# tobiashepp/torch-mednet

Measured on AMD Instinct MI355X. Metric: 128^3 patches/sec training, 3D U-Net 32-base-ch, higher is better.
Workload: dtype bf16; 1 GPU; ResidualUNet3D f_maps=[32, 64, 128, 256] 4-class, 128^3 patches, batch 4/GPU, fwd+DiceLoss+bwd+allreduce+Adam (BASELINE config 2); global_batch=4, parallelism=dp1, graph_replay=False, gradient_exchange=none (1 rank)

## Files before the change

include/mednet_hip.h:

```cpp
#ifndef MEDNET_HIP_H
#define MEDNET_HIP_H
#include <stddef.h>
#include <stdint.h>
#ifdef __cplusplus
extern "C" {
#endif

typedef void* mednet_stream;

enum { MEDNET_F32 = 0, MEDNET_BF16 = 1,
       MEDNET_F16 = 2,
       MEDNET_U8 = 3,
       MEDNET_I64 = 4,
       MEDNET_I16 = 5   };
enum { MEDNET_NDHWC = 0, MEDNET_NCDHW = 1 };
enum { MEDNET_ACT_NONE = 0, MEDNET_ACT_RELU = 1, MEDNET_ACT_LEAKY = 2, MEDNET_ACT_ELU = 3 };
enum { MEDNET_POOL_MAX = 0, MEDNET_POOL_AVG = 1 };
enum { MEDNET_ALGO_AUTO = 0, MEDNET_ALGO_DIRECT = 1, MEDNET_ALGO_MFMA = 2, MEDNET_ALGO_EXACT = 3,
       MEDNET_ALGO_EXACT_BIT = 4,
       MEDNET_ALGO_SPLITW_BIT = 8 };
enum { MEDNET_PACK_LOW = 0x100,
       MEDNET_PACK_HIGH_ONLY = 0x200 };
enum { MEDNET_REG_L2 = 0, MEDNET_REG_L1 = 1 };
enum { MEDNET_CLASS_DICE = 0, MEDNET_CLASS_CE = 1, MEDNET_CLASS_DICE_CE = 2 };
enum {
  MEDNET_OK = 0, MEDNET_E_SHAPE = -1, MEDNET_E_DTYPE = -2, MEDNET_E_WORKSPACE = -3, MEDNET_E_HIP = -4,
  MEDNET_E_UNSUPPORTED = -5
};
#define MEDNET_NO_IGNORE INT32_MIN

int mednet_abi_version(void);
const char* mednet_last_error(void);
int mednet_device_ok(void);
int mednet_set_option(const char* name, int value);
int mednet_get_option(const char* name, int default_value);

size_t mednet_conv3d_pack_bytes(int cin, int cout, int ksize);
int mednet_conv3d_pack_elt(const float* w, void* packed, int cin, int cout, int ksize, int transposed_src, int elt_dtype,
                           mednet_stream stream);
int mednet_conv3d_pack(const float* w, void* packed, int cin, int cout, int ksize, int transposed_src,
                       mednet_stream stream);
typedef struct mednet_pack_job {
  const float* w;
  void* packed;
  int cin, cout, ksize, transposed_src;
} mednet_pack_job;
size_t mednet_conv3d_pack_table_bytes(int njobs);
int mednet_conv3d_pack_table(const mednet_pack_job* jobs, int njobs, void* table_host, unsigned* blocks);
int mednet_conv3d_pack_many(const void* table_device, int njobs, unsigned blocks, int elt_dtype, mednet_stream stream);
int mednet_conv3d_stats_plan(int n, int d, int h, int w, int cin, int cout, int dtype, int gnb, int stride, int* out13);
int mednet_conv3d_fused_stats_chunks(int n, int d, int h, int w, int cin, int cout, int ksize, int x_dtype,
                                     int y_dtype, int algo);
int mednet_conv3d_fwd(const void* x, const void* packed, const float* bias, void* y, int n, int d, int h, int w,
                      int cin, int cout, int ksize, int x_dtype, int x_layout, int y_dtype, int y_layout,
                      int dgrad, int algo, float* gn_partial, mednet_stream stream);
int mednet_conv3d_cm_supported(int cin, int cout, int ksize, int x_dtype, int y_dtype, int algo);
int mednet_conv3d_act_supported(int n, int d, int h, int w, int cin, int cout, int algo);
int mednet_conv3d_act_fwd(const void* x, const void* packed, void* y, int n, int d, int h, int w, int cin, int cout,
                          int act, int algo, float* gn_partial, int dtype, mednet_stream stream);
int mednet_conv3d_dgrad_add(const void* dy, const void* packed, const void* add, void* dx, int n, int d, int h, int w,
                            int cin, int cout, int algo, int dtype, mednet_stream stream);
int mednet_conv3d_dgrad_gn_rows(int n, int d, int h, int w, int cin, int cout, int algo);
int mednet_conv3d_dgrad_gn_rows_dt(int n, int d, int h, int w, int cin, int cout, int algo, int dtype);
int mednet_conv3d_dgrad_add_supported(int n, int d, int h, int w, int cin, int cout, int algo, int dtype);
int mednet_conv3d_dgrad_gn(const void* dy, const void* packed, const void* add, void* dx, const void* gn_y,
                           const float* gn_coef, int gn_act, float* gn_partial, int n, int d, int h, int w, int cin,
                           int cout, int algo, int dtype, mednet_stream stream);
int mednet_head_dgrad_gn_rows(int n, int d, int h, int w, int cin, int dtype);
int mednet_head_dgrad_gn(const void* dy, const void* packed, void* dx, const void* gn_y, const void* gn_z, int gn_act,
                         float* gn_partial, int n, int d, int h, int w, int cin, int cout, int dtype, mednet_stream stream);
int mednet_convt3d_dgrad_gn_rows(int n, int d, int h, int w, int cin, int cout, int dtype, int algo);
int mednet_convt3d_dgrad_gn(const void* dy, const void* packed, void* dx, const void* gn_y, const void* gn_z, int gn_act,
                            float* gn_partial, int n, int d, int h, int w, int cin, int cout, int dtype, int algo,
                            mednet_stream stream);
int mednet_pool2_bwd_gn_rows(int n, int d, int h, int w, int c, int dtype);
int mednet_pool2_bwd_gn(const void* dy, const void* x, const void* add, void* dx, const void* gn_y, int gn_act,
                        float* gn_partial, int n, int d, int h, int w, int c, int mode, int dtype, mednet_stream stream);
size_t mednet_conv3d_wgrad_ws_bytes(int n, int d, int h, int w, int cin, int cout, int ksize, int workgroups);
int mednet_conv3d_wgrad_coresident(int n, int d, int h, int w, int cin, int cout, int ksize, int x_dtype, int dy_dtype, int algo);
int mednet_conv3d_wgrad_plan(int n, int d, int h, int w, int cin, int cout, int dtype, int workgroups, int* out10);
int mednet_conv3d_wgrad_c1_gn_supported(int cout, int x_dtype, int dtype);
int mednet_conv3d_wgrad_c1_gn(const void* x, const void* dz, const void* y, const float* coef, const float* bcoef, float* dw,
                              int n, int d, int h, int w, int cout, int act, int x_dtype, int dtype, void* ws, size_t ws_bytes,
// ... 329 lines not shown
```

torch-mednet_amd/csrc/api.hip:

```cpp
#include <stdarg.h>
#include <string.h>
#include "common.h"
#include "conv.h"

static thread_local char g_err[512] = "";

int mednet_internal_fail(int code, const char* fmt, ...) {
  va_list ap;
  va_start(ap, fmt);
  vsnprintf(g_err, sizeof(g_err), fmt, ap);
  va_end(ap);
  return code;
}
int mednet_internal_check_launch(const char* what) {
  const hipError_t e = hipGetLastError();
  if (e != hipSuccess) return mednet_internal_fail(MEDNET_E_HIP, "%s: %s", what, hipGetErrorString(e));
  return MEDNET_OK;
}

struct Option {
  char name[32];
  int value;
};
static Option g_options[48];
// ... 139 lines not shown
static int conv_common_checks(const char* who, int n, int d, int h, int w, int cin, int cout, int ksize, int dt1, int dt2) {
  MEDNET_REQUIRE(dtype_ok(dt1) && dtype_ok(dt2), MEDNET_E_DTYPE, "%s: bad dtype", who);
  MEDNET_REQUIRE(ksize == 3 || ksize == 1, MEDNET_E_UNSUPPORTED, "%s: kernel size %d (supported: 1, 3)", who, ksize);
  MEDNET_REQUIRE(n > 0 && d > 0 && h > 0 && w > 0 && cin > 0 && cout > 0, MEDNET_E_SHAPE,
                 "%s: bad shape n=%d d=%d h=%d w=%d cin=%d cout=%d", who, n, d, h, w, cin, cout);
  return MEDNET_OK;
}

extern "C" int mednet_conv3d_cm_supported(int cin, int cout, int ksize, int x_dtype, int y_dtype, int algo) {
  if (algo_base(algo) == MEDNET_ALGO_DIRECT || !is16(y_dtype) || !tuning_option("conv_cm", 1)) return 0;
  return cin >= 2 && ELT_CALL(y_dtype, conv_first_mfma_supported, cin, cout, ksize, x_dtype, y_dtype, MEDNET_NDHWC, false) ? 1 : 0;
}

extern "C" int mednet_conv3d_fused_stats_chunks(int n, int d, int h, int w, int cin, int cout, int ksize, int x_dtype,
                                                int y_dtype, int algo) {
  if (algo_base(algo) == MEDNET_ALGO_DIRECT || !tuning_option("conv_fuse_stats", 1)) return 0;
  if (x_dtype == MEDNET_F32 && y_dtype == MEDNET_F32) {
    if (!(algo_f32_mode(algo, x_dtype, y_dtype) && algo_x3(algo))) return 0;
    if (conv_c1_x3_supported(cin, cout, ksize)) return tuning_option("x3_stats", 1) ? conv_c1_x3_stats_rows(d, h, w) : 0;
    return conv_x3_supported(cin, cout, ksize) && conv_x3_fits(d, h, w, cin) ? conv_x3_stats_rows(n, d, h, w, cout) : 0;
  }
  if (cin == 1 ? ELT_CALL(y_dtype, conv_first_mfma_supported, cin, cout, ksize, x_dtype, y_dtype, MEDNET_NDHWC, false)
               : mednet_conv3d_cm_supported(cin, cout, ksize, x_dtype, y_dtype, algo))
    return ELT_CALL(y_dtype, conv_first_stats_chunks, n, d, h, w, cout);
  if (!ELT_CALL(y_dtype, conv_mfma_supported, cin, cout, ksize, x_dtype, y_dtype, MEDNET_NDHWC, MEDNET_NDHWC, false)) return 0;
  return conv_mfma_stats_chunks(n, d, h, w, cin, cout, false, algo_split(algo, y_dtype));
}

extern "C" int mednet_conv3d_stats_plan(int n, int d, int h, int w, int cin, int cout, int dtype, int gnb, int stride, int* out13) {
  MEDNET_REQUIRE(out13 && n > 0 && d > 0 && h > 0 && w > 0 && (stride == 1 || stride == 2), MEDNET_E_SHAPE, "conv3d_stats_plan: bad arguments");
  MEDNET_REQUIRE(is16(dtype) && cin % 16 == 0 && cout % 16 == 0, MEDNET_E_UNSUPPORTED,
                 "conv3d_stats_plan: the 16-bit matrix-core kernels only (dtype %d, %d -> %d)", dtype, cin, cout);
  return ELT_CALL(dtype, conv_mfma_plan, n, d, h, w, cin, cout, (gnb & 1) != 0, stride, out13, (gnb & 2) != 0);
}

extern "C" int mednet_conv3d_fwd(const void* x, const void* packed, const float* bias, void* y, int n, int d, int h,
                                 int w, int cin, int cout, int ksize, int x_dtype, int x_layout, int y_dtype,
                                 int y_layout, int dgrad, int algo, float* gn_partial, mednet_stream stream) {
  int rc = conv_common_checks("conv3d_fwd", n, d, h, w, cin, cout, ksize, x_dtype, y_dtype);
  if (rc) return rc;
  const PackLayout L = dgrad ? pack_layout(cout, cin, ksize) : pack_layout(cin, cout, ksize);
  hipStream_t s = (hipStream_t)stream;
  const bool mfma_ok = ELT_CALL(y_dtype, conv_mfma_supported, cin, cout, ksize, x_dtype, y_dtype, x_layout, y_layout, bias != nullptr) &&
                       conv_mfma_fits(n, d, h, w, cin);
  const bool f32_mode = algo_f32_mode(algo, x_dtype, y_dtype) && ksize == 3 && (x_layout == MEDNET_NDHWC || cin == 1) && y_layout == MEDNET_NDHWC;
  if (!dgrad && !bias && y_layout == MEDNET_NDHWC && (x_layout == MEDNET_NDHWC || x_layout == MEDNET_NCDHW) &&
      mednet_conv3d_cm_supported(cin, cout, ksize, x_dtype, y_dtype, algo))
    return ELT_CALL(y_dtype, launch_conv_first_mfma, x, x_layout, x_dtype, pack_f32(packed, L, 0), y, n, d, h, w, cin, cout,
                    gn_partial, s, algo_split(algo, y_dtype) ? 1 : 0);
  if (algo_base(algo) == MEDNET_ALGO_MFMA && !mfma_ok && !f32_mode)
    return fail(MEDNET_E_UNSUPPORTED, "conv3d_fwd: MFMA path does not take cin=%d cout=%d k=%d dtypes %d->%d", cin, cout,
                ksize, x_dtype, y_dtype);
  if (mfma_ok && algo_base(algo) != MEDNET_ALGO_DIRECT)
    return ELT_CALL(y_dtype, launch_conv_mfma, x, pack_mfma(packed, L, dgrad), y, n, d, h, w, cin, cout, x_dtype,
                    y_dtype, gn_partial, s, MEDNET_ACT_NONE, nullptr, algo_lo_delta(algo, y_dtype, L));
  if (!dgrad && algo_base(algo) != MEDNET_ALGO_DIRECT && x_layout == MEDNET_NDHWC && cin == 1 &&
      ELT_CALL(y_dtype, conv_first_mfma_supported, cin, cout, ksize, x_dtype, y_dtype, y_layout, bias != nullptr))
    return ELT_CALL(y_dtype, launch_conv_first_mfma, x, x_layout, x_dtype, pack_f32(packed, L, 0), y, n, d, h, w, cin, cout,
                    gn_partial, s, algo_split(algo, y_dtype) ? 1 : 0);
  if (f32_mode && algo_x3(algo) && L.mfma_bytes && conv_x3_supported(cin, cout, ksize) && conv_x3_fits(d, h, w, cin))
    return launch_conv_x3(x, pack_mfma(packed, L, dgrad), L.lo_delta, bias, y, n, d, h, w, cin, cout, gn_partial, s);
  if (f32_mode && !dgrad && algo_x3(algo) && conv_c1_x3_supported(cin, cout, ksize))
    return launch_conv_c1_x3(x, pack_f32(packed, L, 0), bias, y, n, d, h, w, cout, gn_partial, s);
  MEDNET_REQUIRE(gn_partial == nullptr, MEDNET_E_UNSUPPORTED,
                 "conv3d_fwd: fused GroupNorm partials are only produced by the MFMA paths (ask mednet_conv3d_fused_stats_chunks)");
  if (f32_mode)
// ... 527 lines not shown
```

torch-mednet_amd/csrc/conv_mfma.hip:

```cpp
#include <type_traits>
#include "conv.h"

#include "elt16.inc"

namespace mednet {

template <int KIND>
struct FwdTile;
template <>
struct FwdTile<1> {
  static constexpr int TZ = 4, TY = 8, TX = 16, STRIDE = 1;
};
template <>
struct FwdTile<2> {
  static constexpr int TZ = 2, TY = 4, TX = 16, STRIDE = 2;
};
template <>
struct FwdTile<3> {
  static constexpr int TZ = 4, TY = 8, TX = 8, STRIDE = 1;
};
static bool narrow_bricks(int w) {
  const int mode = tuning_option("conv_narrow", 1);
  return mode != 0 && (w <= 8 || (mode == 2 && (w + 7) / 8 < 2 * ((w + 15) / 16)));
}
// ... 444 lines not shown
      for (int k = 0; k < 8; ++k) {
        park[k * 256] = ebs[k];
        park[(8 + k) * 256] = ebq[k];
      }
    }
    if (a.gn_partial && !a.stats_accum) flush_any(n, tis * 4 + e_wv, cb);
    if (!has_next) {
      if (a.gn_partial && a.stats_accum) {
        while (acc_n < a.n) {
          flush_any(acc_n, acc_row, cb);
          ++acc_n;
        }
      }
      break;
    }
    cur_bid = nbid;
    ctile = ntile;
    ccb = ncb2;
  }
}

enum : int { C32_GNB = 1, C32_ADD = 2, C32_STATS = 4, C32_ACT = 8, C32_SPLIT = 16  };
#ifdef MEDNET_ELT_F16
#define MEDNET_MFMA_ASM_OP "v_mfma_f32_32x32x16_f16"
#else
#define MEDNET_MFMA_ASM_OP "v_mfma_f32_32x32x16_bf16"
#endif
__device__ __forceinline__ void mfma_a_acc(f32x16& acc, const eltx8& w_in_agpr, const eltx8& b) {
  asm volatile(MEDNET_MFMA_ASM_OP " %0, %1, %2, %0" : "+v"(acc) : "a"(w_in_agpr), "v"(b));
}
__device__ __forceinline__ void mfma_a_zero(f32x16& acc, const eltx8& w_in_agpr, const eltx8& b) {
  asm volatile(MEDNET_MFMA_ASM_OP " %0, %1, %2, 0" : "=v"(acc) : "a"(w_in_agpr), "v"(b));
}
template <int V>
__global__ __launch_bounds__(256, 1) void conv32_mfma_kernel(FwdArgs a) {
  constexpr bool GNB = (V & C32_GNB) != 0, ADD = (V & C32_ADD) != 0, STATS = (V & C32_STATS) != 0, ACT = (V & C32_ACT) != 0;
  static_assert(!(GNB && (STATS || ACT)), "the data-gradient variant has its own sums and no activation");
  constexpr int TZ = 4, TY = 8, TX = 16, HZ = 6, HY = 10, HX = 18, NV = HZ * HY * HX, NTW = 4;
  constexpr int PIECES = 4 * NV, IN_ROUNDS = (PIECES + 255) / 256;
  constexpr int NVP = NV + 4, BUF_PIECES = 4 * NVP;
  typedef __attribute__((ext_vector_type(4))) unsigned u32x4;
  typedef __attribute__((ext_vector_type(2))) elt eltx2;
  extern __shared__ __attribute__((aligned(16))) char smem[];
  u32x4* in_lds = reinterpret_cast<u32x4*>(smem);
  elt* wlds = reinterpret_cast<elt*>(smem + (size_t)2 * BUF_PIECES * 16) + (threadIdx.x >> 6) * 2048;
  const int tid = threadIdx.x, lane = tid & 63, wv = tid >> 6;
  const int r = lane & 31, h = lane >> 5;
  const int wv_s = __builtin_amdgcn_readfirstlane(wv);
  const int xcd = (int)(blockIdx.x & 7);
  auto origin = [&](int q, int& n, int& tz0, int& ty0, int& tx0) {
    if (a.zslab) {
      int qd = fastdiv(q, a.tiles_x, a.rcp_tiles_x);
      tx0 = (q - qd * a.tiles_x) * TX;
      const int yy = fastdiv(qd, a.zslab, a.rcp_zslab);
      const int zz = xcd * a.zslab + (qd - yy * a.zslab);
      ty0 = yy * TY;
      n = fastdiv(zz, a.tiles_z, a.rcp_tiles_z);
      tz0 = (zz - n * a.tiles_z) * TZ;
    } else {
      int tt = a.xcd_chunk ? xcd * a.xcd_chunk + q : q;
      int qd = fastdiv(tt, a.tiles_x, a.rcp_tiles_x);
      tx0 = (tt - qd * a.tiles_x) * TX;
      tt = qd;
      qd = fastdiv(tt, a.tiles_y, a.rcp_tiles_y);
      ty0 = (tt - qd * a.tiles_y) * TY;
      tt = qd;
      qd = fastdiv(tt, a.tiles_z, a.rcp_tiles_z);
// ... 45 lines not shown
  };
  const int seq_step = a.xcd_chunk ? (int)(gridDim.x >> 3) : (int)gridDim.x;
  const int seq_end = a.xcd_chunk ? a.xcd_chunk : a.ntiles;
  int seq = a.xcd_chunk ? (int)(blockIdx.x >> 3) : (int)blockIdx.x;
  if (seq >= seq_end) {
    if constexpr (GNB || STATS)
      for (int nn = 0; nn < a.n; ++nn) flush(nn);
    return;
  }

#ifndef MEDNET_C32_GNB_LDS
#define MEDNET_C32_GNB_LDS 1
#endif
  constexpr bool GNB_LDS = GNB && MEDNET_C32_GNB_LDS;
  constexpr int NSEC = (ADD ? 8 : 0) + (GNB && !GNB_LDS ? 8 : 0);
  constexpr int SEC0 = 54 - 8, WT = NSEC, TW1 = SEC0, TW0 = TW1 - WT;
  eltx8 wreg[54];
  const u32x4* wp = reinterpret_cast<const u32x4*>(a.wpk) + h * 32 + r;
#pragma unroll
  for (int i = 0; i < 54; ++i)
    if (i < TW0 || i >= TW1) wreg[i] = __builtin_bit_cast(eltx8, wp[((i / 27) * 27 + tap_at(i % 27)) * 64]);

  constexpr unsigned OOB = 0xFFFFFF00u;
  constexpr int MAIN_ROUNDS = HZ * HY / 4, TAIL_ROUNDS = 2;
  static_assert(MAIN_ROUNDS * 4 == HZ * HY && MAIN_ROUNDS + TAIL_ROUNDS == IN_ROUNDS && TAIL_ROUNDS * 32 >= HZ * HY, "round layout");
  const int q4 = lane & 3, hx_main = lane >> 2;
  int tail_pos[TAIL_ROUNDS];
#pragma unroll
  for (int k = 0; k < TAIL_ROUNDS; ++k) {
    const int row = 32 * k + (tid >> 3);
    tail_pos[k] = row < HZ * HY ? ((row / HY) << 8) | (row % HY) : 0x7F00;
  }
  const int tail_hx = 16 + ((tid >> 2) & 1);
  u32x4 in_reg[IN_ROUNDS];
  auto rsrc_of = [&](int n, bool ok) {
    return __builtin_amdgcn_make_buffer_rsrc((void*)(a.x + (size_t)n * a.id * a.ih * a.iw * 32), 0, a.bytes_x & (0u - (unsigned)ok), 0x00020000);
  };
  unsigned voff_main = 0;
  auto plan_main = [&](int tx0) {
    const int gx = tx0 - 1 + hx_main;
    voff_main = (unsigned)gx < (unsigned)a.iw ? (unsigned)gx * 64u + (unsigned)q4 * 16u : OOB;
  };
  auto tail_voff = [&](int k, int tz0, int ty0, int tx0) {
    const int gz = tz0 - 1 + (tail_pos[k] >> 8), gy = ty0 - 1 + (tail_pos[k] & 255), gxt = tx0 - 1 + tail_hx;
    const bool ok = ((unsigned)gz < (unsigned)a.id) & ((unsigned)gy < (unsigned)a.ih) & ((unsigned)gxt < (unsigned)a.iw);
    return ok ? (unsigned)((gz * a.ih + gy) * a.iw + gxt) * 64u + (unsigned)q4 * 16u : OOB;
  };
  int lr_gz = 0, lr_gy = 0;
  unsigned lr_soff = 0, lr_num = 0;
  auto load_round = [&](int it, int phase, int n, int tz0, int ty0, int tx0, bool valid) {
    if (it < MAIN_ROUNDS) {
      if (phase == 0 || phase < 0) {
        const int row = it * 4 + wv_s;
        const int hz = (row * 205) >> 11, hy = row - hz * HY;
        lr_gz = tz0 - 1 + hz;
        lr_gy = ty0 - 1 + hy;
      }
      if (phase == 1 || phase < 0) {
        const bool ok = valid & ((unsigned)lr_gz < (unsigned)a.id) & ((unsigned)lr_gy < (unsigned)a.ih);
        lr_num = a.bytes_x & (0u - (unsigned)ok);
      }
      if (phase == 2 || phase < 0) lr_soff = (unsigned)((lr_gz * a.ih + lr_gy) * a.iw) * 64u;
      if (phase == 3 || phase < 0)
        in_reg[it] = __builtin_amdgcn_raw_buffer_load_b128(
            __builtin_amdgcn_make_buffer_rsrc((void*)(a.x + (size_t)n * a.id * a.ih * a.iw * 32), 0, lr_num, 0x00020000), voff_main, lr_soff, 0);
    } else if (phase == 3 || phase < 0) {
      in_reg[it] = __builtin_amdgcn_raw_buffer_load_b128(rsrc_of(n, valid), tail_voff(it - MAIN_ROUNDS, tz0, ty0, tx0), 0, 0);
    }
  };
  const int slot_main = q4 * NVP + hx_main;
  int slot_tail[TAIL_ROUNDS];
#pragma unroll
  for (int k = 0; k < TAIL_ROUNDS; ++k) {
    const int row = 32 * k + (tid >> 3);
    slot_tail[k] = row < HZ * HY ? q4 * NVP + row * HX + tail_hx : -1;
  }
  const int spare_slot = (2 * BUF_PIECES * 16 + 4 * 4096) / 16 + tid;
  auto commit_one = [&](int b, int it) {
    if (it < MAIN_ROUNDS) {
      in_lds[b * BUF_PIECES + (it * 4 + wv_s) * HX + slot_main] = in_reg[it];
    } else {
      const int sl = slot_tail[it - MAIN_ROUNDS];
      in_lds[sl >= 0 ? b * BUF_PIECES + sl : spare_slot] = in_reg[it];
    }
  };
  const int lx6 = ((r & 15) + 8 * (r >> 4)) & 15;
  const int lbase6 = (wv * HY + 4 * (r >> 4)) * HX + lx6;
  [[maybe_unused]] const eltx2 ones = {(elt)1.0f, (elt)1.0f};
  const size_t ovol = (size_t)a.od * a.oh * a.ow;

  {
    int n0, tz0, ty0, tx0;
    origin(seq, n0, tz0, ty0, tx0);
    plan_main(tx0);
#pragma unroll
    for (int it = 0; it < IN_ROUNDS; ++it) load_round(it, -1, n0, tz0, ty0, tx0, true);
#pragma unroll
    for (int it = 0; it < IN_ROUNDS; ++it) commit_one(0, it);
    const bool valid1 = seq + seq_step < seq_end;
    origin(valid1 ? seq + seq_step : 0, n0, tz0, ty0, tx0);
    plan_main(tx0);
#pragma unroll
    for (int it = 0; it < IN_ROUNDS; ++it) load_round(it, -1, n0, tz0, ty0, tx0, valid1);
  }
  int buf = 0;
  [[maybe_unused]] int coef_n = -1;
  [[maybe_unused]] char* cf_lds = smem + (size_t)2 * BUF_PIECES * 16 + 4 * 4096 + wv_s * 256;
  static_assert(4 * 256 <= 224 * 16, "the coefficient copies stay clear of the spare slots in use");
  while (true) {
    int n, tz0, ty0, tx0;
    origin(seq, n, tz0, ty0, tx0);
    const bool has_next = seq + seq_step < seq_end;
    const bool has_next2 = seq + 2 * seq_step < seq_end;
    if constexpr (GNB || STATS) {
      while (acc_n < n) {
        flush(acc_n);
        ++acc_n;
      }
    }
    if constexpr (GNB) {
      if (n != coef_n) {
        coef_n = n;
        const auto rsrc_cf = __builtin_amdgcn_make_buffer_rsrc((void*)(a.gnb_coef + (size_t)n * 64), 0, 256u, 0x00020000);
        const u32x4 c4 = __builtin_amdgcn_raw_buffer_load_b128(rsrc_cf, (unsigned)(lane * 16), 0, 0);
        wave_lds_fence();
        if (lane < 16) *reinterpret_cast<u32x4*>(cf_lds + lane * 16) = c4;
        wave_lds_fence();
      }
    }
    int n2, tz2, ty2, tx2;
    origin(has_next2 ? seq + 2 * seq_step : 0, n2, tz2, ty2, tx2);
    __syncthreads();

    const int pj = lane & 3, ev = lane >> 2;
    const bool plane_ok = tz0 + wv_s < a.od;
    const bool lane_ok = tx0 + ev < a.ow;
    const unsigned vb = lane_ok ? (unsigned)(ev * 32 + pj * 8) * 2u : OOB;
    unsigned row_num[8], row_off[8];
    auto plan_row = [&](int j) {
      const bool ok = plane_ok & (ty0 + j < a.oh);
      row_num[j] = a.bytes_y & (0u - (unsigned)ok);
      row_off[j] = (unsigned)((((tz0 + wv_s) * a.oh + ty0 + j) * a.ow + tx0) * 32) * 2u;
      asm volatile("" : "+s"(row_num[j]), "+s"(row_off[j]));
    };
    auto row_rsrc = [&](const elt* base, int j) {
      return __builtin_amdgcn_make_buffer_rsrc((void*)(base + (size_t)n * ovol * 32), 0, row_num[j], 0x00020000);
    };
    auto row_soff = [&](int j) { return row_off[j]; };
    [[maybe_unused]] eltx8 adr[ADD ? 8 : 1], yrw[GNB ? 8 : 1];
    [[maybe_unused]] char* ydst = reinterpret_cast<char*>(in_lds + (size_t)buf * BUF_PIECES) + wv_s * 8192;
    static_assert(!GNB_LDS || 4 * 8192 <= 2 * NVP * 16, "the four waves' rows fit the two dead planes");

    f32x16 acc[NTW];
    const u32x4* img = in_lds + (size_t)buf * BUF_PIECES;
    auto b_fragment = [&](int gq, int a6) {
      const int kc1 = gq / 9, kz1 = (gq / 3) % 3, kx1 = gq % 3;
      return __builtin_bit_cast(eltx8, img[(2 * kc1 + h) * NVP + lbase6 + (kz1 * HY + a6) * HX + kx1]);
    };
    eltx8 xf[2][6];
#pragma unroll
    for (int a6 = 0; a6 < 6; ++a6) xf[0][a6] = b_fragment(0, a6);
#pragma unroll
    for (int s54 = 0; s54 < 54; ++s54) {
      const int gq = s54 / 3, ky = s54 % 3, cur = gq & 1;
      const int round = s54 / 3;
      const bool staging = s54 % 3 == 0 && round < IN_ROUNDS;
#pragma unroll
      for (int t = 0; t < NTW; ++t) {
        __builtin_amdgcn_sched_barrier(0);
        if (s54 == 0) mfma_a_zero(acc[t], wreg[0], xf[cur][t]);
        else mfma_a_acc(acc[t], wreg[s54], xf[cur][t + ky]);
        __builtin_amdgcn_sched_barrier(0);
        if (gq + 1 < 18 && (t & 1) == 0) xf[cur ^ 1][(ky * 4 + t) >> 1] = b_fragment(gq + 1, (ky * 4 + t) >> 1);
        if (s54 == 0 && t == 1) plan_main(tx2);
        if (t == 3 && s54 >= 24 && s54 < 32) plan_row(s54 - 24);
        if (t == 2 && s54 < WT)
          wreg[TW0 + s54] = __builtin_bit_cast(eltx8, __builtin_nontemporal_load(wp + (((TW0 + s54) / 27) * 27 + tap_at((TW0 + s54) % 27)) * 64));
        if (t == 2 && s54 >= SEC0) {
          const int j = s54 - SEC0;
          if constexpr (ADD) adr[j] = __builtin_bit_cast(eltx8, __builtin_amdgcn_raw_buffer_load_b128(row_rsrc(a.add, j), vb, row_soff(j), 0));
          if constexpr (GNB && !GNB_LDS) yrw[j] = __builtin_bit_cast(eltx8, __builtin_amdgcn_raw_buffer_load_b128(row_rsrc(a.gnb_y, j), vb, row_soff(j), 0));
        }
        if constexpr (GNB_LDS) {
          if (t == 2 && s54 == 27) __builtin_amdgcn_s_barrier();
          if (t == 2 && s54 >= 27 && s54 < 35) {
            const int j = s54 - 27;
            const __amdgpu_buffer_rsrc_t yr = __builtin_amdgcn_make_buffer_rsrc((void*)(a.gnb_y + (size_t)n * ovol * 32), 0, row_num[j], 0x00020000);
            __builtin_amdgcn_raw_ptr_buffer_load_lds(yr, (__attribute__((address_space(3))) void*)(ydst + j * 1024), 16, vb, row_off[j], 0, 0);
          }
        }
        if (staging) {
          if (t == 0) commit_one(buf ^ 1, round);
          load_round(round, t, n2, tz2, ty2, tx2, has_next2);
        }
      }
    }
    __builtin_amdgcn_sched_barrier(0);

    if constexpr (ACT) {
#pragma unroll
      for (int t = 0; t < NTW; ++t) act_apply_v16(acc[t], a.act);
    }
    const int e_lx = lx6;
    const int e_sw = (e_lx >> 1) & 7;
    eltx8 rows[8];
#pragma unroll
    for (int half = 0; half < 2; ++half) {
      wave_lds_fence();
      if ((r >> 4) == half) {
#pragma unroll
        for (int t = 0; t < NTW; ++t) {
          const int vl = t * 16 + e_lx;
#pragma unroll
          for (int q = 0; q < 4; ++q) {
            eltx4 o;
#pragma unroll
            for (int j = 0; j < 4; ++j) o[j] = (elt)acc[t][q * 4 + j];
            *reinterpret_cast<eltx4*>(wlds + vl * 32 + ((2 * q + h) ^ e_sw) * 4) = o;
          }
        }
      }
      wave_lds_fence();
#pragma unroll
      for (int j = 0; j < 4; ++j) {
        const int vox = j * 16 + ev, swl = (vox >> 1) & 7;
        rows[4 * half + j] = *reinterpret_cast<const eltx8*>(wlds + vox * 32 + (pj ^ (swl >> 1)) * 8);
// ... 395 lines not shown
  const size_t fwd_bytes = mfma ? align_up((size_t)27 * ((cout + 31) / 32 * 32) * cin * sizeof(elt), 256) : 0;
  const size_t bwd_bytes = mfma ? align_up((size_t)27 * ((cin + 31) / 32 * 32) * cout * sizeof(elt), 256) : 0;
  L.mfma_bytes = fwd_bytes > bwd_bytes ? fwd_bytes : bwd_bytes;
  L.mfma_fwd = 2 * f32;
  L.mfma_bwd = 2 * f32 + fwd_bytes;
  L.lo_delta = fwd_bytes + bwd_bytes;
  L.total = 2 * f32 + 2 * (fwd_bytes + bwd_bytes) + 256;
  return L;
}

unsigned pack_mfma_blocks(int cin, int cout) { return 2 * pack_img_tiles(cin, cout); }
int launch_pack_mfma(const float* w, void* sec_fwd, void* sec_bwd, float* Pf, float* Pb, int cin, int cout, int T,
                     int transposed_src, hipStream_t s, size_t lo_delta) {
  if (T != 27) return MEDNET_OK;
  hipLaunchKernelGGL(pack_mfma_kernel, dim3(pack_mfma_blocks(cin, cout)), dim3(256), 0, s, w, (elt*)sec_fwd, (elt*)sec_bwd, cout, cin,
                     transposed_src ? 2 : 0, transposed_src ? 3 : 1, Pf, Pb, transposed_src, lo_delta);
  return check_launch("pack_mfma");
}
int launch_pack_mfma_many(const void* table_device, int njobs, unsigned max_blocks, hipStream_t s, int with_low) {
  hipLaunchKernelGGL(pack_mfma_many_kernel, dim3(max_blocks), dim3(256), 0, s, (const PackJobDev*)table_device, njobs, with_low);
  return check_launch("pack_mfma_many");
}

bool conv_mfma_fits(int n, int d, int h, int w, int c) {
  (void)n;
  return (double)d * h * w * c * 2.0 < 4294960000.0;
}
bool conv_mfma_supported(int cin, int cout, int ksize, int x_dtype, int y_dtype, int x_layout, int y_layout, bool bias) {
  return ksize == 3 && cin % 16 == 0 && cout % 16 == 0 && x_dtype == ELT_DTYPE && y_dtype == ELT_DTYPE &&
         x_layout == MEDNET_NDHWC && y_layout == MEDNET_NDHWC && !bias;
}

static bool conv32_applies(int ntiles, int cin, int cout) {
  return cin == 32 && cout == 32 && ntiles >= 512 && ::mednet_internal_cu_count() == 256 && tuning_option("conv32", 1);
}
static bool conv32_takes(int ntiles, int cin, int cout, bool gnb, bool split = false) {
  return !split && conv32_applies(ntiles, cin, cout) && (!gnb || tuning_option("conv32_gnb", 1));
}
static bool conv2b_takes(int ntiles, int cin, int cout, bool split = false) {
  if (split) return cout % 32 == 0 && cin % 16 == 0 && ::mednet_internal_cu_count() == 256 && tuning_option("conv2b_split", 1);
  if (!(cout % 64 == 0 && cin % 16 == 0 && cin >= tuning_option("conv2b_min_cin", 64) && ::mednet_internal_cu_count() == 256 &&
        tuning_option("conv2b", 1)))
    return false;
  const int nitems = ((ntiles + 7) / 8) * 8 * (cout / 64);
  const int rounds = (nitems + 255) / 256;
  return nitems >= 256 && nitems * 100 >= tuning_option("conv2b_min_fill", 80) * rounds * 256;
}
static int conv_fwd_kind(int n, int d, int h, int w, int cin, int cout, bool gnb, bool split = false) {
  return narrow_bricks(w) && !conv32_takes(bricks<FwdTile<1>>(n, d, h, w), cin, cout, gnb, split) ? 3 : 1;
}
static int conv2b_grid(int nitems) { return nitems < 256 ? nitems : 256; }
static bool convt_dgrad32_takes(int ntiles, int k_dy, int m_dx, bool split) {
  return k_dy == 32 && m_dx == 64 && !split && ntiles >= 256 && ::mednet_internal_cu_count() == 256 && tuning_option("convt_dgrad32", 1);
}
static void conv_stats_plan(int n, int d, int h, int w, int cin, int cout, int& rows, int& accum, bool gnb = false, bool split = false) {
  const int tx = conv_fwd_kind(n, d, h, w, cin, cout, gnb, split) == 3 ? FwdTile<3>::TX : FwdTile<1>::TX;
  using G = FwdTile<1>;
  const int tps = bricks<G>(1, d, h, w, tx);
  const int ncb = (cout + 31) / 32, ntiles = n * tps;
  if (tx == G::TX && conv32_takes(ntiles, cin, cout, gnb, split)) {
    accum = 1;
    rows = 256 * 4;
    return;
  }
  if (tx == G::TX && conv2b_takes(ntiles, cin, cout, split)) {
    const int ncbp = split ? cout / 32 : cout / 64;
    const int grid = conv2b_grid(((ntiles + 7) / 8) * 8 * ncbp);
    accum = tuning_option("conv_stats_accum", 1) && ntiles % 8 == 0 && (grid / 8) % ncbp == 0;
// ... 92 lines not shown
  a.rcp_zslab = 0;
  if constexpr (KIND == 2) {
    if (convt_dgrad32_takes(a.ntiles, cin, cout, split) && !add && act == MEDNET_ACT_NONE) {
      Ct32Args c;
      c.dy = a.x; c.wpk = a.wpk; c.dx = a.y;
      c.gn_y = a.gnb_y; c.gn_z = a.gnb_z; c.gn_partial = a.gn_partial; c.gn_act = a.gnb_act;
      c.n = n; c.d = od; c.h = oh; c.w = ow;
      c.tiles_z = a.tiles_z; c.tiles_y = a.tiles_y; c.tiles_x = a.tiles_x; c.ntiles = a.ntiles;
      c.rcp_tiles_x = a.rcp_tiles_x; c.rcp_tiles_y = a.rcp_tiles_y; c.rcp_tiles_z = a.rcp_tiles_z;
      c.bytes_dy = a.bytes_x; c.bytes_dx = a.bytes_y;
      const int rows32 = 2 * 256;
      if (probe) {
        a.stats_accum = 1;
        a.stats_rows = rows32;
        a.xcd_chunk = a.ntiles % 8 == 0 ? a.ntiles / 8 : 0;
        return plan_answer(probe, 7, 256, a.ntiles, a);
      }
      return launch_lds("convt_dgrad32_mfma", use_gnb ? convt_dgrad32_mfma_kernel<true> : convt_dgrad32_mfma_kernel<false>, dim3(256), dim3(256),
                        CT32_LDS, s, c);
    }
  }
  if constexpr (KIND == 1) {
    const int variant = c32_variant(use_gnb, add != nullptr, gn_partial != nullptr, act != MEDNET_ACT_NONE, split);
    if (conv32_takes(a.ntiles, cin, cout, use_gnb, split)) {
      constexpr size_t lds32 = (size_t)2 * 4 * (HZ * HY * HX + 4) * 16 + 4 * 4096 + 256 * 16;
      static_assert(lds32 <= 160 * 1024, "two bricks of whole rows + the waves' epilogue areas + spare slots");
      a.xcd_chunk = a.ntiles % 8 == 0 ? a.ntiles / 8 : 0;
      if ((n * a.tiles_z) % 8 == 0 && a.tiles_z % (n * a.tiles_z / 8) == 0 && tuning_option("conv32_zslab", 1)) {
        a.zslab = n * a.tiles_z / 8;
        a.rcp_zslab = fastdiv_rcp(a.zslab);
      }
      MEDNET_REQUIRE(!use_gnb || act == MEDNET_ACT_NONE, MEDNET_E_UNSUPPORTED, "conv32_mfma: no activation in the data-gradient form");
      if (probe) return plan_answer(probe, 4, 256, a.ntiles, a);
      return c32_dispatch(variant, [&](auto v) {
        return launch_lds("conv32_mfma", conv32_mfma_kernel<decltype(v)::value>, dim3(256), dim3(256), lds32, s, a);
      });
    }
    if (conv2b_takes(a.ntiles, cin, cout, split)) {
      FwdArgs b2 = a;
      b2.ncb = split ? cout / 32 : cout / 64;
      b2.rcp_ncb = fastdiv_rcp(b2.ncb);
      b2.nitems = ((a.ntiles + 7) / 8) * 8 * b2.ncb;
      b2.nkc = a.nkc_in;
      b2.xcd_chunk = (a.ntiles % 8 == 0 && tuning_option("conv2b_xcd_walk", 1)) ? a.ntiles / 8 : 0;
      const int grid2 = conv2b_grid(b2.nitems);
      MEDNET_REQUIRE(!use_gnb || act == MEDNET_ACT_NONE, MEDNET_E_UNSUPPORTED, "conv2b_mfma: no activation in the data-gradient form");
      if (probe) return plan_answer(probe, b2.stats_accum ? 6 : 5, grid2, b2.nitems, b2);
      return c32_dispatch(variant, [&](auto v) {
        constexpr int V = decltype(v)::value;
        return launch_lds("conv2b_mfma", split ? conv2b_mfma_kernel<V | C32_SPLIT> : conv2b_mfma_kernel<V>, dim3(grid2), dim3(256), C2B_LDS, s, b2);
      });
    }
  }
  if (probe) return plan_answer(probe, a.stats_accum ? 3 : 2, (int)grid, a.nitems, a);
  if constexpr (STRIDE == 1) {
    if (use_gnb) {
      constexpr size_t lds_gnb = lds + 16 * 256 * sizeof(float);
      static_assert(lds_gnb <= 80 * 1024, "two workgroups must fit one CU");
      return launch_lds("conv_mfma(gnb)", conv_mfma_kernel<KIND, true>, dim3(grid), dim3(256), lds_gnb, s, a);
    }
  }
  if constexpr (STRIDE == 2) {
    if (use_gnb) return launch_lds("conv_mfma(gnb, stride 2)", conv_mfma_kernel<2, true>, dim3(grid), dim3(256), lds, s, a);
  }
  return launch_lds("conv_mfma", conv_mfma_kernel<KIND>, dim3(grid), dim3(256), lds, s, a);
}

static int fwd_by_kind(const void* x, const void* sec, void* y, int n, int d, int h, int w, int cin, int cout, float* gn_partial,
// ... 10 lines not shown
  return fwd_by_kind(x, packed_section, y, n, d, h, w, cin, cout, gn_partial, s, act, add, GnbSpec(), nullptr, lo_delta);
}
int launch_conv_mfma_gnb(const void* dy, const void* packed_section, void* dx, int n, int d, int h, int w, int cin, int cout,
                         const void* add, const void* gn_y, const float* gn_coef, int gn_act, float* gn_partial, hipStream_t s,
                         size_t lo_delta) {
  GnbSpec g;
  g.y = gn_y;
  g.coef = gn_coef;
  g.act = gn_act;
  return fwd_by_kind(dy, packed_section, dx, n, d, h, w, cin, cout, gn_partial, s, MEDNET_ACT_NONE, add, g, nullptr, lo_delta);
}
int conv_mfma_plan(int n, int d, int h, int w, int cin, int cout, bool gnb, int stride, int* out, bool split) {
  FwdPlanProbe p{};
  const size_t lo = split ? 256 : 0;
  float dummy_partial;
  GnbSpec g;
  int rc;
  if (stride == 2) {
    g.y = g.z = &dummy_partial;
    rc = launch_fwd<2>(nullptr, nullptr, nullptr, n, d, h, w, 2 * d, 2 * h, 2 * w, cout, cin, &dummy_partial, nullptr, MEDNET_ACT_NONE,
                       nullptr, g, &p, lo);
  } else {
    if (gnb) {
      g.y = &dummy_partial;
      g.coef = &dummy_partial;
    }
    rc = fwd_by_kind(nullptr, nullptr, nullptr, n, d, h, w, cin, cout, &dummy_partial, nullptr, MEDNET_ACT_NONE, nullptr, g, &p, lo);
  }
  if (rc) return rc;
  const int v[13] = {p.kind, p.grid, p.nitems, p.ncb, p.ntiles, p.tiles_per_sample, p.accum, p.rows, p.xcd_chunk, p.zslab,
                     p.tiles_x, p.tiles_y, p.tiles_z};
  for (int i = 0; i < 13; ++i) out[i] = v[i];
  return MEDNET_OK;
}
int conv_mfma_stats_chunks(int n, int d, int h, int w, int cin, int cout, bool gnb, bool split) {
  int rows, accum;
  conv_stats_plan(n, d, h, w, cin, cout, rows, accum, gnb, split);
  if (gnb && !tuning_option("conv_fuse_gnb_general", 1) && !conv32_takes(bricks<FwdTile<1>>(n, d, h, w), cin, cout, true, split)) return 0;
  return rows;
}

int launch_convt_dgrad_mfma(const void* dy, const void* packed_section, void* dx, int n, int d, int h, int w, int cin,
                            int cout, hipStream_t s, size_t lo_delta) {
  return launch_fwd<2>(dy, packed_section, dx, n, d, h, w, 2 * d, 2 * h, 2 * w, cout, cin, nullptr, s, MEDNET_ACT_NONE, nullptr, GnbSpec(),
                       nullptr, lo_delta);
}
int convt_dgrad_gn_rows(int n, int d, int h, int w, int cin, int cout, bool split) {
  const int tps = bricks<FwdTile<2>>(1, d, h, w);
  if (convt_dgrad32_takes(n * tps, cout, cin, split)) return 2 * 256;
  return 4 * tps;
}
int launch_convt_dgrad_gn_mfma(const void* dy, const void* packed_section, void* dx, const void* gn_y, const void* gn_z, int gn_act,
                               float* gn_partial, int n, int d, int h, int w, int cin, int cout, hipStream_t s, size_t lo_delta) {
  GnbSpec g;
  g.y = gn_y;
  g.z = gn_z;
  g.act = gn_act;
  return launch_fwd<2>(dy, packed_section, dx, n, d, h, w, 2 * d, 2 * h, 2 * w, cout, cin, gn_partial, s, MEDNET_ACT_NONE, nullptr, g,
                       nullptr, lo_delta);
}

struct Wg2Args {
  const elt* A;
  const elt* B;
  float* part;
  int n, d, h, w, ka, kb;
// ... 725 lines not shown
```

torch-mednet_amd/csrc/conv_mfma_decl.inc:

```
struct PackLayout {
  int taps;
  size_t f32_fwd, f32_bwd;
  size_t mfma_fwd, mfma_bwd;
  size_t mfma_bytes;
  size_t lo_delta;
  size_t total;
};
PackLayout pack_layout(int cin, int cout, int ksize);
struct PackJobDev {
  const float* w;
  void* sec_fwd;
  void* sec_bwd;
  float* Pf;
  float* Pb;
  int cin, cout, transposed;
  unsigned nblocks;
  int lo_delta;
  unsigned first_block;
};
bool conv_mfma_fits(int n, int d, int h, int w, int c);
bool conv_mfma_supported(int cin, int cout, int ksize, int x_dtype, int y_dtype, int x_layout, int y_layout, bool bias);
int launch_conv_mfma(const void* x, const void* packed_section, void* y, int n, int d, int h, int w, int cin, int cout,
                     int x_dtype, int y_dtype, float* gn_partial, hipStream_t s, int act = MEDNET_ACT_NONE,
                     const void* add = nullptr, size_t lo_delta = 0);
int launch_conv_mfma_gnb(const void* dy, const void* packed_section, void* dx, int n, int d, int h, int w, int cin, int cout,
                         const void* add, const void* gn_y, const float* gn_coef, int gn_act, float* gn_partial, hipStream_t s,
                         size_t lo_delta = 0);
int conv_mfma_plan(int n, int d, int h, int w, int cin, int cout, bool gnb, int stride, int* out, bool split = false);
int conv_mfma_stats_chunks(int n, int d, int h, int w, int cin, int cout, bool gnb = false, bool split = false);
int launch_pack_mfma(const float* w, void* sec_fwd, void* sec_bwd, float* Pf, float* Pb, int cin, int cout, int T,
                     int transposed_src, hipStream_t s, size_t lo_delta = 0);
unsigned pack_mfma_blocks(int cin, int cout);
int launch_pack_mfma_many(const void* table_device, int njobs, unsigned max_blocks, hipStream_t s, int with_low = 0);
bool wgrad_mfma_supported(int cin, int cout, int ksize, int x_dtype, int dy_dtype, int x_layout, int dy_layout);
bool wgrad_mfma_fits(int n, int d, int h, int w, int cmax, int scale);
bool wgrad_mfma_coresident(int d, int h, int w);
int wgrad_mfma_plan(int n, int d, int h, int w, int cin, int cout, int workgroups, int* out);
size_t wgrad_mfma_ws_bytes(int n, int d, int h, int w, int cin, int cout, int ksize, int workgroups);
int launch_wgrad_mfma(const void* x, const void* dy, float* dw, int n, int d, int h, int w, int cin, int cout, int dtype,
                      void* ws, size_t ws_bytes, hipStream_t s, int workgroups);
int launch_convt_fwd_mfma(const void* x, const void* sec, const float* bias, const void* skip, void* y, int n, int d,
                          int h, int w, int cin, int cout, hipStream_t s, size_t lo_delta = 0);
int launch_convt_dgrad_mfma(const void* dy, const void* packed_section, void* dx, int n, int d, int h, int w, int cin,
                            int cout, hipStream_t s, size_t lo_delta = 0);
int convt_dgrad_gn_rows(int n, int d, int h, int w, int cin, int cout, bool split = false);
int launch_convt_dgrad_gn_mfma(const void* dy, const void* packed_section, void* dx, const void* gn_y, const void* gn_z, int gn_act,
                               float* gn_partial, int n, int d, int h, int w, int cin, int cout, hipStream_t s, size_t lo_delta = 0);
size_t convt_wgrad_mfma_ws_bytes(int n, int d, int h, int w, int cin, int cout, int workgroups);
int launch_convt_wgrad_mfma(const void* x, const void* dy, float* dw, int n, int d, int h, int w, int cin, int cout,
                            void* ws, size_t ws_bytes, hipStream_t s, int workgroups);

bool conv_first_mfma_supported(int cin, int cout, int ksize, int x_dtype, int y_dtype, int y_layout, bool bias);
int conv_first_stats_chunks(int n, int d, int h, int w, int cout);
int launch_conv_first_mfma(const void* x, int x_layout, int x_dtype, const float* w_pf, void* y, int n, int d, int h, int w, int cin,
                           int cout, float* gn_partial, hipStream_t s, int split = 0);
bool wgrad_first_mfma_supported(int cin, int cout, int x_dtype, int dy_dtype);
void wgrad_first_mfma_plan(int n, int d, int h, int w, int cin, int cout, bool gn, int* out4);
int wgrad_first_mfma_blocks(int n, int d, int h, int w, int cin, int cout, bool gn);
int launch_wgrad_first_mfma(const void* x, int x_layout, int x_dtype, const void* dy, float* part, int n, int d, int h, int w, int cin,
                            int cout, hipStream_t s, const void* gn_y = nullptr, const float* gn_coef = nullptr,
                            const float* gn_bcoef = nullptr, int gn_act = 0);
// ... 33 lines not shown
```

torch-mednet_amd/mednet_hip/_lib.py:

```python
from __future__ import annotations

import ctypes as C
import os

import torch

_HERE = os.path.dirname(os.path.abspath(__file__))
LIB_PATH = os.environ.get("MEDNET_LIB_PATH") or os.path.join(_HERE, "libmednet_hip.so")

F32, BF16 = 0, 1
NDHWC, NCDHW = 0, 1
ACT_NONE, ACT_RELU, ACT_LEAKY, ACT_ELU = 0, 1, 2, 3
POOL_MAX, POOL_AVG = 0, 1
ALGO_AUTO, ALGO_DIRECT, ALGO_MFMA, ALGO_EXACT = 0, 1, 2, 3
ALGO_EXACT_BIT = 4
ALGO_SPLITW_BIT = 8
PACK_LOW = 0x100
PACK_HIGH_ONLY = 0x200
REG_L2, REG_L1 = 0, 1
CLASS_DICE, CLASS_CE, CLASS_DICE_CE = 0, 1, 2
PAD_CONSTANT, PAD_SYMMETRIC = 0, 1
MIP_MEAN, MIP_MAX = 0, 1
BLEND_PROBABILITIES, BLEND_LOGITS = 0, 1
INTERP_LINEAR, INTERP_NEAREST = 0, 1
BORDER_CONSTANT, BORDER_EDGE = 0, 1
F16, U8, I64 = 2, 3, 4
I16 = 5
INTENSITY_MAX_RANKS, INTENSITY_TABLE_BYTES = 8, 40
INTENSITY_ALL, INTENSITY_FIRST, INTENSITY_LAST = -1, 1, 2
INTENSITY_ZSCORE, INTENSITY_CT, INTENSITY_RESCALE, INTENSITY_PERCENTILES = 0, 1, 2, 3
NO_IGNORE = -(2 ** 31)
CC_ALL = -1

_vp, _i, _sz, _f, _i64, _dbl = C.c_void_p, C.c_int, C.c_size_t, C.c_float, C.c_int64, C.c_double

SIGNATURES = {
    "mednet_abi_version": (_i, []),
    "mednet_last_error": (C.c_char_p, []),
    "mednet_device_ok": (_i, []),
    "mednet_set_option": (_i, [C.c_char_p, _i]),
    "mednet_get_option": (_i, [C.c_char_p, _i]),
    "mednet_conv3d_pack_bytes": (_sz, [_i, _i, _i]),
    "mednet_conv3d_pack": (_i, [_vp, _vp, _i, _i, _i, _i, _vp]),
    "mednet_conv3d_pack_elt": (_i, [_vp, _vp, _i, _i, _i, _i, _i, _vp]),
    "mednet_conv3d_pack_table_bytes": (_sz, [_i]),
    "mednet_conv3d_pack_table": (_i, [_vp, _i, _vp, _vp]),
    "mednet_conv3d_pack_many": (_i, [_vp, _i, C.c_uint, _i, _vp]),
    "mednet_conv3d_stats_plan": (_i, [_i] * 9 + [_vp]),
    "mednet_conv3d_fused_stats_chunks": (_i, [_i] * 10),
    "mednet_conv3d_fwd": (_i, [_vp, _vp, _vp, _vp] + [_i] * 13 + [_vp, _vp]),
    "mednet_gn_finalize": (_i, [_vp, _i, _vp, _vp, _vp, _vp, _i, _sz, _i, _i, _f, _vp, _sz, _vp]),
    "mednet_conv3d_act_supported": (_i, [_i] * 7),
    "mednet_conv3d_act_fwd": (_i, [_vp, _vp, _vp] + [_i] * 8 + [_vp, _i, _vp]),
    "mednet_conv3d_dgrad_add": (_i, [_vp, _vp, _vp, _vp] + [_i] * 8 + [_vp]),
    "mednet_conv3d_dgrad_gn_rows": (_i, [_i] * 7),
    "mednet_conv3d_dgrad_gn_rows_dt": (_i, [_i] * 8),
    "mednet_conv3d_dgrad_add_supported": (_i, [_i] * 8),
    "mednet_conv3d_dgrad_gn": (_i, [_vp, _vp, _vp, _vp, _vp, _vp, _i, _vp] + [_i] * 8 + [_vp]),
    "mednet_gn_act_bwd_fused": (_i, [_vp] * 6 + [_i, _vp, _vp, _vp, _i, _sz, _i, _i, _i, _i, _i, _vp, _sz, _vp]),
    "mednet_gn_bwd_coefficients": (_i, [_vp, _vp, _vp, _i, _vp, _vp, _vp, _i, _sz, _i, _i, _vp, _sz, _vp]),
    "mednet_gn_act_bwd_fused_res": (_i, [_vp] * 7 + [_i, _vp, _vp, _vp, _vp, _i, _sz, _i, _i, _i, _i, _vp, _sz, _vp]),
    "mednet_gn_act_bwd_fused_res_pool": (_i, [_vp] * 7 + [_i, _vp, _vp, _vp, _vp] + [_i] * 9 + [_vp, _sz, _vp]),
    "mednet_gn_act_bwd_fused_res_head_supported": (_i, [_i] * 4),
    "mednet_gn_act_bwd_fused_res_head": (_i, [_vp, _vp, _i, _i64] + [_vp] * 4 + [_f, _i, _i, _i, _i] + [_vp] * 5 + [_i, _vp, _vp, _vp, _vp,
                                              _i, _sz, _i, _i, _i, _i, _vp, _sz, _vp]),
    "mednet_head_dgrad_gn_rows": (_i, [_i] * 6),
    "mednet_head_dgrad_gn": (_i, [_vp] * 5 + [_i, _vp] + [_i] * 7 + [_vp]),
    "mednet_pool2_bwd_gn_rows": (_i, [_i] * 6),
    "mednet_convt3d_dgrad_gn_rows": (_i, [_i] * 8),
    "mednet_convt3d_dgrad_gn": (_i, [_vp] * 5 + [_i, _vp] + [_i] * 8 + [_vp]),
    "mednet_pool2_bwd_gn": (_i, [_vp] * 5 + [_i, _vp] + [_i] * 7 + [_vp]),
    "mednet_conv3d_wgrad_ws_bytes": (_sz, [_i] * 8),
    "mednet_conv3d_wgrad_coresident": (_i, [_i] * 10),
    "mednet_conv3d_wgrad_plan": (_i, [_i] * 8 + [_vp]),
    "mednet_conv3d_wgrad_c1_gn_supported": (_i, [_i] * 3),
    "mednet_conv3d_wgrad_c1_gn": (_i, [_vp] * 6 + [_i] * 8 + [_vp, _sz, _vp]),
    "mednet_conv3d_cm_supported": (_i, [_i] * 6),
    "mednet_conv3d_wgrad_cm_gn_supported": (_i, [_i] * 4),
    "mednet_conv3d_wgrad_cm_plan": (_i, [_i] * 8 + [_vp]),
    "mednet_conv3d_wgrad_cm_gn": (_i, [_vp, _i] + [_vp] * 5 + [_i] * 9 + [_vp, _sz, _vp]),
    "mednet_conv3d_wgrad": (_i, [_vp, _vp, _vp, _vp] + [_i] * 13 + [_vp, _sz, _vp]),
# ... 190 lines not shown
```

Baseline: 212.0 patches/s.

## Stage conv32 input halo tiles via direct buffer-to-LDS loads

Adds a DMA variant of the 32->32 channel MFMA conv kernel that loads input halo bricks straight into LDS with buffer_load_lds instead of going through registers and explicit LDS stores. Halo bounds are handled by a packed-coordinate guard test that sends out-of-range lanes to an OOB offset. Prefetch depth drops from two tiles ahead to one, with a vmcnt wait before the barrier. The variant is on by default through a tuning option. The intent is to cut VGPR pressure and LDS store instructions, at the cost of less prefetch lookahead.

```diff
diff --git a/include/mednet_hip.h b/include/mednet_hip.h
--- a/include/mednet_hip.h
+++ b/include/mednet_hip.h
@@ -49,6 +49,7 @@
 int mednet_conv3d_pack_table(const mednet_pack_job* jobs, int njobs, void* table_host, unsigned* blocks);
 int mednet_conv3d_pack_many(const void* table_device, int njobs, unsigned blocks, int elt_dtype, mednet_stream stream);
 int mednet_conv3d_stats_plan(int n, int d, int h, int w, int cin, int cout, int dtype, int gnb, int stride, int* out13);
+int mednet_conv32_form(int n, int d, int h, int w, int dtype, int gnb);
 int mednet_conv3d_fused_stats_chunks(int n, int d, int h, int w, int cin, int cout, int ksize, int x_dtype,
                                      int y_dtype, int algo);
 int mednet_conv3d_fwd(const void* x, const void* packed, const float* bias, void* y, int n, int d, int h, int w,
diff --git a/torch-mednet_amd/csrc/api.hip b/torch-mednet_amd/csrc/api.hip
--- a/torch-mednet_amd/csrc/api.hip
+++ b/torch-mednet_amd/csrc/api.hip
@@ -195,6 +195,11 @@
   MEDNET_REQUIRE(is16(dtype) && cin % 16 == 0 && cout % 16 == 0, MEDNET_E_UNSUPPORTED,
                  "conv3d_stats_plan: the 16-bit matrix-core kernels only (dtype %d, %d -> %d)", dtype, cin, cout);
   return ELT_CALL(dtype, conv_mfma_plan, n, d, h, w, cin, cout, (gnb & 1) != 0, stride, out13, (gnb & 2) != 0);
+}
+
+extern "C" int mednet_conv32_form(int n, int d, int h, int w, int dtype, int gnb) {
+  MEDNET_REQUIRE(n > 0 && d > 0 && h > 0 && w > 0 && is16(dtype), MEDNET_E_SHAPE, "conv32_form: bad arguments");
+  return ELT_CALL(dtype, conv32_form, n, d, h, w, gnb != 0);
 }
 
 extern "C" int mednet_conv3d_fwd(const void* x, const void* packed, const float* bias, void* y, int n, int d, int h,
diff --git a/torch-mednet_amd/csrc/conv_mfma.hip b/torch-mednet_amd/csrc/conv_mfma.hip
--- a/torch-mednet_amd/csrc/conv_mfma.hip
+++ b/torch-mednet_amd/csrc/conv_mfma.hip
@@ -500,7 +500,7 @@
 __device__ __forceinline__ void mfma_a_zero(f32x16& acc, const eltx8& w_in_agpr, const eltx8& b) {
   asm volatile(MEDNET_MFMA_ASM_OP " %0, %1, %2, 0" : "=v"(acc) : "a"(w_in_agpr), "v"(b));
 }
-template <int V>
+template <int V, bool DMA>
 __global__ __launch_bounds__(256, 1) void conv32_mfma_kernel(FwdArgs a) {
   constexpr bool GNB = (V & C32_GNB) != 0, ADD = (V & C32_ADD) != 0, STATS = (V & C32_STATS) != 0, ACT = (V & C32_ACT) != 0;
   static_assert(!(GNB && (STATS || ACT)), "the data-gradient variant has its own sums and no activation");
@@ -612,7 +612,7 @@
     tail_pos[k] = row < HZ * HY ? ((row / HY) << 8) | (row % HY) : 0x7F00;
   }
   const int tail_hx = 16 + ((tid >> 2) & 1);
-  u32x4 in_reg[IN_ROUNDS];
+  [[maybe_unused]] u32x4 in_reg[DMA ? 1 : IN_ROUNDS];
   auto rsrc_of = [&](int n, bool ok) {
     return __builtin_amdgcn_make_buffer_rsrc((void*)(a.x + (size_t)n * a.id * a.ih * a.iw * 32), 0, a.bytes_x & (0u - (unsigned)ok), 0x00020000);
   };
@@ -642,10 +642,10 @@
       }
       if (phase == 2 || phase < 0) lr_soff = (unsigned)((lr_gz * a.ih + lr_gy) * a.iw) * 64u;
       if (phase == 3 || phase < 0)
-        in_reg[it] = __builtin_amdgcn_raw_buffer_load_b128(
+        in_reg[DMA ? 0 : it] = __builtin_amdgcn_raw_buffer_load_b128(
             __builtin_amdgcn_make_buffer_rsrc((void*)(a.x + (size_t)n * a.id * a.ih * a.iw * 32), 0, lr_num, 0x00020000), voff_main, lr_soff, 0);
     } else if (phase == 3 || phase < 0) {
-      in_reg[it] = __builtin_amdgcn_raw_buffer_load_b128(rsrc_of(n, valid), tail_voff(it - MAIN_ROUNDS, tz0, ty0, tx0), 0, 0);
+      in_reg[DMA ? 0 : it] = __builtin_amdgcn_raw_buffer_load_b128(rsrc_of(n, valid), tail_voff(it - MAIN_ROUNDS, tz0, ty0, tx0), 0, 0);
     }
   };
   const int slot_main = q4 * NVP + hx_main;
@@ -658,10 +658,42 @@
   const int spare_slot = (2 * BUF_PIECES * 16 + 4 * 4096) / 16 + tid;
   auto commit_one = [&](int b, int it) {
     if (it < MAIN_ROUNDS) {
-      in_lds[b * BUF_PIECES + (it * 4 + wv_s) * HX + slot_main] = in_reg[it];
+      in_lds[b * BUF_PIECES + (it * 4 + wv_s) * HX + slot_main] = in_reg[DMA ? 0 : it];
     } else {
       const int sl = slot_tail[it - MAIN_ROUNDS];
-      in_lds[sl >= 0 ? b * BUF_PIECES + sl : spare_slot] = in_reg[it];
+      in_lds[sl >= 0 ? b * BUF_PIECES + sl : spare_slot] = in_reg[DMA ? 0 : it];
+    }
+  };
+  constexpr unsigned DGUARD = 0x00808080u;
+  [[maybe_unused]] unsigned dpos[DMA ? IN_ROUNDS : 1], drel[DMA ? IN_ROUNDS : 1];
+  if constexpr (DMA) {
+#pragma unroll
+    for (int k = 0; k < IN_ROUNDS; ++k) {
+      const int v = (64 * k < NV - 64 ? 64 * k : NV - 64) + lane;
+      const int hz = v / (HY * HX), hy = (v / HX) % HY, hx = v % HX;
+      dpos[k] = (unsigned)((hz << 16) | (hy << 8) | hx);
+      drel[k] = (unsigned)((hz * a.ih + hy) * a.iw + hx) * 64u + (unsigned)wv * 16u;
+    }
+  }
+  [[maybe_unused]] unsigned d_lo = 0, d_hi = 0, d_off = 0, d_num = 0, d_t = 0, d_voff = 0;
+  [[maybe_unused]] int d_n = 0;
+  auto plan_dma = [&](int n, int tz0, int ty0, int tx0, bool valid) {
+    const int zlo = tz0 < 1 ? 1 - tz0 : 0, ylo = ty0 < 1 ? 1 - ty0 : 0, xlo = tx0 < 1 ? 1 - tx0 : 0;
+    const int zhi = a.id - tz0 < HZ - 1 ? a.id - tz0 : HZ - 1, yhi = a.ih - ty0 < HY - 1 ? a.ih - ty0 : HY - 1,
+              xhi = a.iw - tx0 < HX - 1 ? a.iw - tx0 : HX - 1;
+    d_lo = (unsigned)(((128 - zlo) << 16) | ((128 - ylo) << 8) | (128 - xlo));
+    d_hi = (unsigned)(((128 + zhi) << 16) | ((128 + yhi) << 8) | (128 + xhi));
+    d_off = (unsigned)(((tz0 - 1) * a.ih + (ty0 - 1)) * a.iw + (tx0 - 1)) * 64u;
+    d_num = a.bytes_x & (0u - (unsigned)valid);
+    d_n = n;
+  };
+  auto dma_round = [&](int it, int phase, int b) {
+    if (phase == 0 || phase < 0) d_t = (dpos[DMA ? it : 0] + d_lo) & (d_hi - dpos[DMA ? it : 0]) & DGUARD;
+    if (phase == 1 || phase < 0) d_voff = d_t == DGUARD ? drel[DMA ? it : 0] + d_off : OOB;
+    if (phase == 3 || phase < 0) {
+      const __amdgpu_buffer_rsrc_t xr = __builtin_amdgcn_make_buffer_rsrc((void*)(a.x + (size_t)d_n * a.id * a.ih * a.iw * 32), 0, d_num, 0x00020000);
+      char* dst = smem + (size_t)(((b * 4 + wv_s) * NVP + (64 * it < NV - 64 ? 64 * it : NV - 64)) * 16);
+      __builtin_amdgcn_raw_ptr_buffer_load_lds(xr, (__attribute__((address_space(3))) void*)dst, 16, d_voff, 0, 0, 0);
     }
   };
   const int lx6 = ((r & 15) + 8 * (r >> 4)) & 15;
@@ -669,7 +701,13 @@
   [[maybe_unused]] const eltx2 ones = {(elt)1.0f, (elt)1.0f};
   const size_t ovol = (size_t)a.od * a.oh * a.ow;
 
-  {
+  if constexpr (DMA) {
+    int n0, tz0, ty0, tx0;
+    origin(seq, n0, tz0, ty0, tx0);
+    plan_dma(n0, tz0, ty0, tx0, true);
+#pragma unroll
+    for (int it = 0; it < IN_ROUNDS; ++it) dma_round(it, -1, 0);
+  } else {
     int n0, tz0, ty0, tx0;
     origin(seq, n0, tz0, ty0, tx0);
     plan_main(tx0);
@@ -709,7 +747,13 @@
       }
     }
     int n2, tz2, ty2, tx2;
-    origin(has_next2 ? seq + 2 * seq_step : 0, n2, tz2, ty2, tx2);
+    if constexpr (DMA) {
+      origin(has_next ? seq + seq_step : 0, n2, tz2, ty2, tx2);
+      plan_dma(n2, tz2, ty2, tx2, has_next);
+      asm volatile("s_waitcnt vmcnt(0)" ::: "memory");
+    } else {
+      origin(has_next2 ? seq + 2 * seq_step : 0, n2, tz2, ty2, tx2);
+    }
     __syncthreads();
 
     const int pj = lane & 3, ev = lane >> 2;
@@ -752,7 +796,7 @@
         else mfma_a_acc(acc[t], wreg[s54], xf[cur][t + ky]);
         __builtin_amdgcn_sched_barrier(0);
         if (gq + 1 < 18 && (t & 1) == 0) xf[cur ^ 1][(ky * 4 + t) >> 1] = b_fragment(gq + 1, (ky * 4 + t) >> 1);
-        if (s54 == 0 && t == 1) plan_main(tx2);
+        if (!DMA && s54 == 0 && t == 1) plan_main(tx2);
         if (t == 3 && s54 >= 24 && s54 < 32) plan_row(s54 - 24);
         if (t == 2 && s54 < WT)
           wreg[TW0 + s54] = __builtin_bit_cast(eltx8, __builtin_nontemporal_load(wp + (((TW0 + s54) / 27) * 27 + tap_at((TW0 + s54) % 27)) * 64));
@@ -770,8 +814,12 @@
           }
         }
         if (staging) {
-          if (t == 0) commit_one(buf ^ 1, round);
-          load_round(round, t, n2, tz2, ty2, tx2, has_next2);
+          if constexpr (DMA) {
+            dma_round(round, t, buf ^ 1);
+          } else {
+            if (t == 0) commit_one(buf ^ 1, round);
+            load_round(round, t, n2, tz2, ty2, tx2, has_next2);
+          }
         }
       }
     }
@@ -1233,8 +1281,10 @@
 }
 
 static bool conv32_applies(int ntiles, int cin, int cout) {
-  return cin == 32 && cout == 32 && ntiles >= 512 && ::mednet_internal_cu_count() == 256 && tuning_option("conv32", 1);
-}
+  return cin == 32 && cout == 32 && ntiles >= tuning_option("conv32_min_bricks", 512) && ::mednet_internal_cu_count() == 256 &&
+         tuning_option("conv32", 1);
+}
+static bool conv32_dma() { return tuning_option("conv32_dma", 1) != 0; }
 static bool conv32_takes(int ntiles, int cin, int cout, bool gnb, bool split = false) {
   return !split && conv32_applies(ntiles, cin, cout) && (!gnb || tuning_option("conv32_gnb", 1));
 }
@@ -1393,8 +1443,10 @@
       }
       MEDNET_REQUIRE(!use_gnb || act == MEDNET_ACT_NONE, MEDNET_E_UNSUPPORTED, "conv32_mfma: no activation in the data-gradient form");
       if (probe) return plan_answer(probe, 4, 256, a.ntiles, a);
+      const bool dma = conv32_dma();
       return c32_dispatch(variant, [&](auto v) {
-        return launch_lds("conv32_mfma", conv32_mfma_kernel<decltype(v)::value>, dim3(256), dim3(256), lds32, s, a);
+        constexpr int V = decltype(v)::value;
+        return launch_lds("conv32_mfma", dma ? conv32_mfma_kernel<V, true> : conv32_mfma_kernel<V, false>, dim3(256), dim3(256), lds32, s, a);
       });
     }
     if (conv2b_takes(a.ntiles, cin, cout, split)) {
@@ -1471,6 +1523,10 @@
                      p.tiles_x, p.tiles_y, p.tiles_z};
   for (int i = 0; i < 13; ++i) out[i] = v[i];
   return MEDNET_OK;
+}
+int conv32_form(int n, int d, int h, int w, bool gnb) {
+  if (conv_fwd_kind(n, d, h, w, 32, 32, gnb) != 1 || !conv32_takes(bricks<FwdTile<1>>(n, d, h, w), 32, 32, gnb)) return 3;
+  return conv32_dma() ? 1 : 0;
 }
 int conv_mfma_stats_chunks(int n, int d, int h, int w, int cin, int cout, bool gnb, bool split) {
   int rows, accum;
diff --git a/torch-mednet_amd/csrc/conv_mfma_decl.inc b/torch-mednet_amd/csrc/conv_mfma_decl.inc
--- a/torch-mednet_amd/csrc/conv_mfma_decl.inc
+++ b/torch-mednet_amd/csrc/conv_mfma_decl.inc
@@ -27,6 +27,7 @@
                          const void* add, const void* gn_y, const float* gn_coef, int gn_act, float* gn_partial, hipStream_t s,
                          size_t lo_delta = 0);
 int conv_mfma_plan(int n, int d, int h, int w, int cin, int cout, bool gnb, int stride, int* out, bool split = false);
+int conv32_form(int n, int d, int h, int w, bool gnb);
 int conv_mfma_stats_chunks(int n, int d, int h, int w, int cin, int cout, bool gnb = false, bool split = false);
 int launch_pack_mfma(const float* w, void* sec_fwd, void* sec_bwd, float* Pf, float* Pb, int cin, int cout, int T,
                      int transposed_src, hipStream_t s, size_t lo_delta = 0);
diff --git a/torch-mednet_amd/mednet_hip/_lib.py b/torch-mednet_amd/mednet_hip/_lib.py
--- a/torch-mednet_amd/mednet_hip/_lib.py
+++ b/torch-mednet_amd/mednet_hip/_lib.py
@@ -47,6 +47,7 @@
     "mednet_conv3d_pack_table": (_i, [_vp, _i, _vp, _vp]),
     "mednet_conv3d_pack_many": (_i, [_vp, _i, C.c_uint, _i, _vp]),
     "mednet_conv3d_stats_plan": (_i, [_i] * 9 + [_vp]),
+    "mednet_conv32_form": (_i, [_i] * 6),
     "mednet_conv3d_fused_stats_chunks": (_i, [_i] * 10),
     "mednet_conv3d_fwd": (_i, [_vp, _vp, _vp, _vp] + [_i] * 13 + [_vp, _vp]),
     "mednet_gn_finalize": (_i, [_vp, _i, _vp, _vp, _vp, _vp, _i, _sz, _i, _i, _f, _vp, _sz, _vp]),
```

New measurement: 213.4 patches/s (median of 6 runs). Within noise of the previous version (+0.6%).
